# createamind/Distributed-DRL

Hardware: AMD Instinct MI355X
Metric: env-steps/s + learner updates/s, SAC1 LunarLanderContinuous-v2 @1/2/4/8 GPU (higher is better)
Workload: dtype f32

## Files before the change

distributed-drl_amd/csrc/loop.hip:

```cpp
#include "ddrl_common.h"

#include <cstdlib>
#include <cstring>
#include <vector>

int ddrl_sac1_internal_opt_sync(ddrl_sac1_t *h, void *stream);
int ddrl_sac1_internal_sample_into(ddrl_sac1_t *h, ddrl_replay_t *replay, int set, void *stream);

struct ddrl_loop {
    ddrl_sac1_t *learner;
    ddrl_replay_t *replay;
    int per_graph;
    uint32_t seed;
    float *buf[2][8];
    int batch;
    hipGraphExec_t exec;
    bool captured;
    int parity;
};

static int sample_into(ddrl_loop *h, int set, void *stream) {
    return ddrl_sac1_internal_sample_into(h->learner, h->replay, set, stream);
}

static int update_from(ddrl_loop *h, int set, void *stream) {
    float **b = h->buf[set];
    int rc = ddrl_sac1_fill_noise(h->learner, h->seed, stream);
    if (rc != DDRL_OK) return rc;
    return ddrl_sac1_step(h->learner, b[0], b[1], b[2], b[3], b[4], b[5], b[6], b[7], nullptr, nullptr, nullptr, nullptr, stream);
}

static int one_update(ddrl_loop *h, void *stream) {
    const int set = h->parity;
    h->parity ^= 1;
    int rc = sample_into(h, set, stream);
    if (rc != DDRL_OK) return rc;
    return update_from(h, set, stream);
}

static int grads_from(ddrl_loop *h, int set, void *stream) {
    float **b = h->buf[set];
    int rc = ddrl_sac1_fill_noise(h->learner, h->seed, stream);
    if (rc != DDRL_OK) return rc;
    return ddrl_sac1_compute_grads(h->learner, b[0], b[1], b[2], b[3], b[4], b[5], b[6], b[7], nullptr, nullptr, nullptr, nullptr,
                                   stream);
}

static int capture(ddrl_loop *h, hipStream_t main_s) {
    const char *fk = getenv("DDRL_LOOP_FORK");
    const int mode = !fk ? 0 : (strcmp(fk, "all") == 0 ? 2 : 1);
    hipStream_t side = nullptr;
    DDRL_HIP_CHECK(hipStreamCreateWithFlags(&side, hipStreamNonBlocking));
    const int n = h->per_graph;
    std::vector<hipEvent_t> e_smp(n + 1), e_upd(n + 1), e_grad(n + 1);
    hipEvent_t e_fork;
    DDRL_HIP_CHECK(hipEventCreateWithFlags(&e_fork, hipEventDisableTiming));
    for (int i = 0; i <= n; ++i) {
        DDRL_HIP_CHECK(hipEventCreateWithFlags(&e_smp[i], hipEventDisableTiming));
        DDRL_HIP_CHECK(hipEventCreateWithFlags(&e_upd[i], hipEventDisableTiming));
        DDRL_HIP_CHECK(hipEventCreateWithFlags(&e_grad[i], hipEventDisableTiming));
    }
    hipGraph_t graph = nullptr;
    int rc = ddrl_sac1_internal_opt_sync(h->learner, (void *)main_s);
    if (rc != DDRL_OK) return rc;
    DDRL_HIP_CHECK(hipStreamSynchronize(main_s));
    DDRL_HIP_CHECK(hipStreamBeginCapture(main_s, hipStreamCaptureModeThreadLocal));
    hipError_t e = hipSuccess;
#define HE(x) do { if (e == hipSuccess && rc == DDRL_OK) e = (x); } while (0)
#define RC(x) do { if (e == hipSuccess && rc == DDRL_OK) rc = (x); } while (0)
    if (mode == 0) {
        RC(sample_into(h, 0, (void *)main_s));
        for (int i = 0; i < n; ++i) {
            RC(ddrl_sac1_fill_noise(h->learner, h->seed, (void *)main_s));
            if (i + 1 < n) {
                RC(ddrl_sac1_step_and_sample(h->learner, i & 1, h->replay, (i + 1) & 1, (void *)main_s));
            } else {
                float **b = h->buf[i & 1];
                RC(ddrl_sac1_step(h->learner, b[0], b[1], b[2], b[3], b[4], b[5], b[6], b[7], nullptr, nullptr, nullptr, nullptr,
                                  (void *)main_s));
            }
        }
    } else if (mode == 2) {
        HE(hipEventRecord(e_fork, main_s));
        HE(hipStreamWaitEvent(side, e_fork, 0));
        for (int i = 0; i < n; ++i) {
            if (i >= 2) HE(hipStreamWaitEvent(side, e_upd[i - 2], 0));
            RC(sample_into(h, i & 1, (void *)side));
            HE(hipEventRecord(e_smp[i], side));
            HE(hipStreamWaitEvent(main_s, e_smp[i], 0));
            RC(update_from(h, i & 1, (void *)main_s));
            HE(hipEventRecord(e_upd[i], main_s));
        }
    } else {
        RC(sample_into(h, 0, (void *)main_s));
        for (int i = 0; i < n; ++i) {
            RC(grads_from(h, i & 1, (void *)main_s));
            if (i + 1 < n) {
                HE(hipEventRecord(e_grad[i], main_s));
                HE(hipStreamWaitEvent(side, e_grad[i], 0));
                RC(sample_into(h, (i + 1) & 1, (void *)side));
                HE(hipEventRecord(e_smp[i + 1], side));
            }
            RC(ddrl_sac1_apply_grads(h->learner, (void *)main_s));
            if (i + 1 < n) HE(hipStreamWaitEvent(main_s, e_smp[i + 1], 0));
        }
    }
    RC(ddrl_sac1_internal_opt_sync(h->learner, (void *)main_s));
#undef HE
#undef RC
    hipError_t e2 = hipStreamEndCapture(main_s, &graph);
    for (int i = 0; i <= n; ++i) { (void)hipEventDestroy(e_smp[i]); (void)hipEventDestroy(e_upd[i]); (void)hipEventDestroy(e_grad[i]); }
    (void)hipEventDestroy(e_fork);
    (void)hipStreamDestroy(side);
    if (rc != DDRL_OK) { if (graph) (void)hipGraphDestroy(graph); return rc; }
    if (e != hipSuccess || e2 != hipSuccess) {
        ddrl::set_error("graph capture failed: %s", hipGetErrorString(e != hipSuccess ? e : e2));
        if (graph) (void)hipGraphDestroy(graph);
        return DDRL_ERR_HIP;
    }
    DDRL_HIP_CHECK(hipGraphInstantiate(&h->exec, graph, nullptr, nullptr, 0));
    (void)hipGraphDestroy(graph);
    h->captured = true;
    return DDRL_OK;
}

extern "C" {

int ddrl_loop_create(ddrl_loop_t **out, ddrl_sac1_t *learner, ddrl_replay_t *replay, int32_t updates_per_graph,
                     uint32_t noise_seed) {
    DDRL_REQUIRE(out && learner && replay, "NULL pointer");
    DDRL_REQUIRE(updates_per_graph >= 0 && updates_per_graph <= 4096, "updates_per_graph must be in [0, 4096]");
    ddrl_loop *h = new ddrl_loop();
    h->learner = learner; h->replay = replay; h->per_graph = updates_per_graph; h->seed = noise_seed;
    h->exec = nullptr; h->captured = false; h->parity = 0;
    int rc = ddrl_sac1_input_buffers(learner, 0, h->buf[0]);
    if (rc == DDRL_OK) rc = ddrl_sac1_input_buffers(learner, 1, h->buf[1]);
    if (rc != DDRL_OK) { delete h; return rc; }
    h->batch = ddrl_sac1_batch(learner);
    *out = h;
    return DDRL_OK;
}

int ddrl_loop_destroy(ddrl_loop_t *h) {
    if (!h) return DDRL_OK;
    if (h->exec) (void)hipGraphExecDestroy(h->exec);
    delete h;
    return DDRL_OK;
}

int ddrl_loop_run(ddrl_loop_t *h, int64_t n_updates, void *stream) {
    DDRL_REQUIRE(h != nullptr && n_updates >= 0, "bad handle / n_updates");
    hipStream_t s = ddrl::as_stream(stream);
    int64_t left = n_updates;
    if (h->per_graph > 0 && left >= h->per_graph) {
        if (!h->captured) {
            int rc = one_update(h, stream);
            if (rc != DDRL_OK) return rc;
            left -= 1;
            hipStream_t cs = s, own = nullptr;
            if (cs == nullptr) {
                DDRL_HIP_CHECK(hipStreamCreateWithFlags(&own, hipStreamNonBlocking));
                DDRL_HIP_CHECK(hipDeviceSynchronize());
                cs = own;
            }
            rc = capture(h, cs);
            if (own) (void)hipStreamDestroy(own);
            if (rc != DDRL_OK) return rc;
        }
        if (left >= h->per_graph) {
            const int rc2 = ddrl_sac1_internal_opt_sync(h->learner, stream);
            if (rc2 != DDRL_OK) return rc2;
        }
        while (left >= h->per_graph) {
            DDRL_HIP_CHECK(hipGraphLaunch(h->exec, s));
            left -= h->per_graph;
        }
    }
    for (; left > 0; --left) {
        int rc = one_update(h, stream);
        if (rc != DDRL_OK) return rc;
    }
    return DDRL_OK;
}

}
```

Baseline: 44430.

## Capture power-of-two graph family with chained sample prefetch across launches

Instead of one graph of per_graph updates with per-update eager fallback for the remainder, capture a family of graphs with lengths per_graph and descending powers of two, each in variants for whether the first sample was already prefetched, which buffer set it starts on, and whether the tail samples ahead for the next graph. The remainder updates are covered by a few graph launches instead of many individual kernel launches, and consecutive graphs chain the prefetched sample so no redundant sample is needed at boundaries. It costs more capture and instantiation time and memory for up to eight variants per length, and adds state-tracking complexity in the launch loop.

```diff
diff --git a/distributed-drl_amd/csrc/loop.hip b/distributed-drl_amd/csrc/loop.hip
--- a/distributed-drl_amd/csrc/loop.hip
+++ b/distributed-drl_amd/csrc/loop.hip
@@ -14,7 +14,9 @@
     uint32_t seed;
     float *buf[2][8];
     int batch;
-    hipGraphExec_t exec;
+    struct Graph { int len; hipGraphExec_t exec[2][2][2]; };
+    std::vector<Graph> family;
+    bool chain;
     bool captured;
     int parity;
 };
@@ -46,16 +48,36 @@
                                    stream);
 }
 
-static int capture(ddrl_loop *h, hipStream_t main_s) {
+static int fork_mode() {
     const char *fk = getenv("DDRL_LOOP_FORK");
-    const int mode = !fk ? 0 : (strcmp(fk, "all") == 0 ? 2 : 1);
+    return !fk ? 0 : (strcmp(fk, "all") == 0 ? 2 : 1);
+}
+
+static bool variant_needed(const ddrl_loop *h, int len, int pre, int start, int tail) {
+    if (!h->chain) return !pre && !start && !tail;
+    if (start && (!pre || (h->per_graph & 1) == 0)) return false;
+    if (tail && len == 1 && h->per_graph != 1) return false;
+    return true;
+}
+
+static void destroy_family(ddrl_loop *h) {
+    for (auto &g : h->family)
+        for (int v = 0; v < 8; ++v)
+            if (g.exec[v >> 2][(v >> 1) & 1][v & 1]) (void)hipGraphExecDestroy(g.exec[v >> 2][(v >> 1) & 1][v & 1]);
+    h->family.clear();
+    h->captured = false;
+}
+
+static int capture(ddrl_loop *h, hipStream_t main_s, int n, int mode, int pre, int start, int tail, hipGraphExec_t *exec) {
     hipStream_t side = nullptr;
-    DDRL_HIP_CHECK(hipStreamCreateWithFlags(&side, hipStreamNonBlocking));
-    const int n = h->per_graph;
-    std::vector<hipEvent_t> e_smp(n + 1), e_upd(n + 1), e_grad(n + 1);
-    hipEvent_t e_fork;
-    DDRL_HIP_CHECK(hipEventCreateWithFlags(&e_fork, hipEventDisableTiming));
-    for (int i = 0; i <= n; ++i) {
+    const int n_ev = mode != 0 ? n + 1 : 0;
+    std::vector<hipEvent_t> e_smp(n_ev), e_upd(n_ev), e_grad(n_ev);
+    hipEvent_t e_fork = nullptr;
+    if (mode != 0) {
+        DDRL_HIP_CHECK(hipStreamCreateWithFlags(&side, hipStreamNonBlocking));
+        DDRL_HIP_CHECK(hipEventCreateWithFlags(&e_fork, hipEventDisableTiming));
+    }
+    for (int i = 0; i < n_ev; ++i) {
         DDRL_HIP_CHECK(hipEventCreateWithFlags(&e_smp[i], hipEventDisableTiming));
         DDRL_HIP_CHECK(hipEventCreateWithFlags(&e_upd[i], hipEventDisableTiming));
         DDRL_HIP_CHECK(hipEventCreateWithFlags(&e_grad[i], hipEventDisableTiming));
@@ -69,13 +91,14 @@
 #define HE(x) do { if (e == hipSuccess && rc == DDRL_OK) e = (x); } while (0)
 #define RC(x) do { if (e == hipSuccess && rc == DDRL_OK) rc = (x); } while (0)
     if (mode == 0) {
-        RC(sample_into(h, 0, (void *)main_s));
+        if (!pre) RC(sample_into(h, start, (void *)main_s));
         for (int i = 0; i < n; ++i) {
+            const int set = (start + i) & 1;
             RC(ddrl_sac1_fill_noise(h->learner, h->seed, (void *)main_s));
-            if (i + 1 < n) {
-                RC(ddrl_sac1_step_and_sample(h->learner, i & 1, h->replay, (i + 1) & 1, (void *)main_s));
+            if (i + 1 < n || tail) {
+                RC(ddrl_sac1_step_and_sample(h->learner, set, h->replay, set ^ 1, (void *)main_s));
             } else {
-                float **b = h->buf[i & 1];
+                float **b = h->buf[set];
                 RC(ddrl_sac1_step(h->learner, b[0], b[1], b[2], b[3], b[4], b[5], b[6], b[7], nullptr, nullptr, nullptr, nullptr,
                                   (void *)main_s));
             }
@@ -109,17 +132,40 @@
 #undef HE
 #undef RC
     hipError_t e2 = hipStreamEndCapture(main_s, &graph);
-    for (int i = 0; i <= n; ++i) { (void)hipEventDestroy(e_smp[i]); (void)hipEventDestroy(e_upd[i]); (void)hipEventDestroy(e_grad[i]); }
-    (void)hipEventDestroy(e_fork);
-    (void)hipStreamDestroy(side);
+    for (int i = 0; i < n_ev; ++i) { (void)hipEventDestroy(e_smp[i]); (void)hipEventDestroy(e_upd[i]); (void)hipEventDestroy(e_grad[i]); }
+    if (e_fork) (void)hipEventDestroy(e_fork);
+    if (side) (void)hipStreamDestroy(side);
     if (rc != DDRL_OK) { if (graph) (void)hipGraphDestroy(graph); return rc; }
     if (e != hipSuccess || e2 != hipSuccess) {
         ddrl::set_error("graph capture failed: %s", hipGetErrorString(e != hipSuccess ? e : e2));
         if (graph) (void)hipGraphDestroy(graph);
         return DDRL_ERR_HIP;
     }
-    DDRL_HIP_CHECK(hipGraphInstantiate(&h->exec, graph, nullptr, nullptr, 0));
+    const hipError_t e3 = hipGraphInstantiate(exec, graph, nullptr, nullptr, 0);
     (void)hipGraphDestroy(graph);
+    if (e3 != hipSuccess) {
+        *exec = nullptr;
+        ddrl::set_error("hipGraphInstantiate failed: %s", hipGetErrorString(e3));
+        return DDRL_ERR_HIP;
+    }
+    return DDRL_OK;
+}
+
+static int capture_family(ddrl_loop *h, hipStream_t main_s) {
+    const int mode = fork_mode();
+    h->chain = mode == 0;
+    h->family.clear();
+    h->family.push_back(ddrl_loop::Graph{h->per_graph, {}});
+    int p = 1;
+    while (p * 2 < h->per_graph) p *= 2;
+    for (; p >= 1 && p < h->per_graph; p >>= 1) h->family.push_back(ddrl_loop::Graph{p, {}});
+    for (auto &g : h->family)
+        for (int v = 0; v < 8; ++v) {
+            const int pre = v >> 2, start = (v >> 1) & 1, tail = v & 1;
+            if (!variant_needed(h, g.len, pre, start, tail)) continue;
+            const int rc = capture(h, main_s, g.len, g.len == h->per_graph ? mode : 0, pre, start, tail, &g.exec[pre][start][tail]);
+            if (rc != DDRL_OK) { destroy_family(h); return rc; }
+        }
     h->captured = true;
     return DDRL_OK;
 }
@@ -132,7 +178,7 @@
     DDRL_REQUIRE(updates_per_graph >= 0 && updates_per_graph <= 4096, "updates_per_graph must be in [0, 4096]");
     ddrl_loop *h = new ddrl_loop();
     h->learner = learner; h->replay = replay; h->per_graph = updates_per_graph; h->seed = noise_seed;
-    h->exec = nullptr; h->captured = false; h->parity = 0;
+    h->chain = false; h->captured = false; h->parity = 0;
     int rc = ddrl_sac1_input_buffers(learner, 0, h->buf[0]);
     if (rc == DDRL_OK) rc = ddrl_sac1_input_buffers(learner, 1, h->buf[1]);
     if (rc != DDRL_OK) { delete h; return rc; }
@@ -143,7 +189,7 @@
 
 int ddrl_loop_destroy(ddrl_loop_t *h) {
     if (!h) return DDRL_OK;
-    if (h->exec) (void)hipGraphExecDestroy(h->exec);
+    destroy_family(h);
     delete h;
     return DDRL_OK;
 }
@@ -152,7 +198,7 @@
     DDRL_REQUIRE(h != nullptr && n_updates >= 0, "bad handle / n_updates");
     hipStream_t s = ddrl::as_stream(stream);
     int64_t left = n_updates;
-    if (h->per_graph > 0 && left >= h->per_graph) {
+    if (h->per_graph > 0 && (h->captured || left >= h->per_graph)) {
         if (!h->captured) {
             int rc = one_update(h, stream);
             if (rc != DDRL_OK) return rc;
@@ -163,18 +209,27 @@
                 DDRL_HIP_CHECK(hipDeviceSynchronize());
                 cs = own;
             }
-            rc = capture(h, cs);
+            rc = capture_family(h, cs);
             if (own) (void)hipStreamDestroy(own);
             if (rc != DDRL_OK) return rc;
         }
-        if (left >= h->per_graph) {
+        if (left > 0) {
             const int rc2 = ddrl_sac1_internal_opt_sync(h->learner, stream);
             if (rc2 != DDRL_OK) return rc2;
         }
-        while (left >= h->per_graph) {
-            DDRL_HIP_CHECK(hipGraphLaunch(h->exec, s));
-            left -= h->per_graph;
-        }
+        bool first = true;
+        int set = 0;
+        for (const auto &g : h->family)
+            while (left >= g.len) {
+                const int pre = (!first && h->chain) ? 1 : 0, tail = (h->chain && left > g.len) ? 1 : 0;
+                if (!pre) set = 0;
+                hipGraphExec_t exec = g.exec[pre][set][tail];
+                DDRL_REQUIRE(exec != nullptr, "no captured graph for this replay (internal)");
+                DDRL_HIP_CHECK(hipGraphLaunch(exec, s));
+                set ^= g.len & 1;
+                left -= g.len;
+                first = false;
+            }
     }
     for (; left > 0; --left) {
         int rc = one_update(h, stream);
```

Result: faster. 45130 (median of 6 runs) (+1.6%).
